# HueCodes/sudoku-vision

Measured on AMD Instinct MI355X. Metric: end-to-end frames/sec (1080p->81 digits), higher is better.
Workload: dtype f32

## Files before the change

sudoku-vision_amd/csrc/k3_cnn.hip:

```cpp
#include <cstring>

#include "sv_device.h"
#include "sv_internal.h"

typedef float f32x4 __attribute__((ext_vector_type(4)));
typedef float f32x2 __attribute__((ext_vector_type(2)));

namespace {

constexpr int PLANE = 257;
constexpr int C1_CELL = 32 * PLANE;
constexpr int IN_W = 30, IN_CELL = 900;
constexpr int FEAT = 3136;

__device__ __forceinline__ float glue_norm(u8 c) { return sv_glue_norm(c); }

struct N1Scratch {
    float cf[784];
    float rw[784];
    unsigned bits[16][8];
    unsigned pre[16][8];
    int residual[16], step[16];
};

// ... 794 lines not shown
    __shared__ N1Scratch sc[4];
    __shared__ float tile[4][IN_CELL];
    const int lane = threadIdx.x & 63, wave = threadIdx.x >> 6;
    const long c = (long)blockIdx.x * 4 + wave;
    if (c >= B) return;
    n1_preprocess_cell(cells + c * 784, tile[wave], sc[wave], lane, taps.k);
    wave_lds_fence();
    for (int i = lane; i < 784; i += 64) {
        const int y = i / 28, x = i - 28 * y;
        out[c * 784 + i] = tile[wave][(y + 1) * IN_W + x + 1] < 0.f ? 255 : 0;
    }
}

}

int svk_pack_weights_f32mfma(sv_weights &w, const float *c2w, const float *f1w)
{
    std::vector<float> w2(2 * 2 * 72 * 64);
    for (int np = 0; np < 2; np++)
        for (int t = 0; t < 2; t++)
            for (int ks = 0; ks < 72; ks++)
                for (int lane = 0; lane < 64; lane++) {
                    const int oc = 32 * np + 16 * t + (lane & 15), tap = ks >> 3, ic = (ks & 7) + 8 * (lane >> 4);
                    w2[((np * 2 + t) * 72 + ks) * 64 + lane] = c2w[(oc * 32 + ic) * 9 + tap];
                }
    std::vector<float> f1((size_t)196 * 8 * 64 * 4);
    for (int c = 0; c < 196; c++)
        for (int t = 0; t < 8; t++)
            for (int lane = 0; lane < 64; lane++)
                for (int e = 0; e < 4; e++) {
                    const int kp = 16 * c + 4 * (lane >> 4) + e, win = kp >> 6, oc = kp & 63, n = 16 * t + (lane & 15);
                    f1[(((size_t)c * 8 + t) * 64 + lane) * 4 + e] = f1w[(size_t)n * 3136 + oc * 49 + win];
                }
    int rc;
    if ((rc = sv_upload(w, &w.conv2_wreg, w2.data(), w2.size()))) return rc;
    if ((rc = sv_upload(w, &w.fc1_wreg, f1.data(), f1.size()))) return rc;
#ifdef SV_XCHECK
    std::vector<float> wino((size_t)4 * 16 * 8 * 64);
    std::vector<uint16_t> wsplit((size_t)4 * 16 * 3 * 64 * 8);
    const double G[4][3] = {{1, 0, 0}, {0.5, 0.5, 0.5}, {0.5, -0.5, 0.5}, {0, 0, 1}};
    for (int oc = 0; oc < 64; oc++)
        for (int ic = 0; ic < 32; ic++) {
            const float *g = c2w + (oc * 32 + ic) * 9;
            double Gg[4][3], U[4][4];
            for (int i = 0; i < 4; i++)
                for (int j = 0; j < 3; j++) Gg[i][j] = G[i][0] * g[j] + G[i][1] * g[3 + j] + G[i][2] * g[6 + j];
            for (int i = 0; i < 4; i++)
                for (int j = 0; j < 4; j++) U[i][j] = Gg[i][0] * G[j][0] + Gg[i][1] * G[j][1] + Gg[i][2] * G[j][2];
            const int nt = oc >> 4, lane = (oc & 15) + 16 * (ic & 3), ks = ic >> 2;
            for (int xi = 0; xi < 16; xi++) {
                const float u = (float)U[xi >> 2][xi & 3];
                wino[(((size_t)nt * 16 + xi) * 8 + ks) * 64 + lane] = u;
                float rest = u;
                for (int part = 0; part < 3; part++) {
                    uint32_t bits;
                    memcpy(&bits, &rest, 4);
                    bits &= 0xffff0000u;
                    float piece;
                    memcpy(&piece, &bits, 4);
                    rest -= piece;
                    wsplit[((((size_t)nt * 16 + xi) * 3 + part) * 64 + (oc & 15) + 16 * (ic >> 3)) * 8 + (ic & 7)] = (uint16_t)(bits >> 16);
                }
            }
        }
    if ((rc = sv_upload(w, &w.conv2_wino, wino.data(), wino.size()))) return rc;
    if ((rc = sv_upload(w, &w.conv2_wsplit, wsplit.data(), wsplit.size()))) return rc;
#endif
    return SV_OK;
}

int svk_preprocess_cells(const u8 *cells, long B, u8 *out, hipStream_t s)
{
    GaussTaps taps;
    sv_gaussian_taps_f32(11, taps.k);
    hipLaunchKernelGGL(k_preprocess_cells, dim3((unsigned)((B + 3) / 4)), dim3(256), 0, s, cells, B, taps, out);
    SV_LAUNCH_CHECK("k_preprocess_cells");
    return SV_OK;
}

__global__ __launch_bounds__(256) void k_softmax_topk(const float *__restrict__ logits, long B, int k, u8 *__restrict__ index, float *__restrict__ prob)
{
    const long cell = (long)blockIdx.x * 256 + threadIdx.x;
    if (cell >= B) return;
    float p[10];
    float best = -INFINITY;
#pragma unroll
    for (int j = 0; j < 10; j++) { p[j] = logits[cell * 10 + j]; best = fmaxf(best, p[j]); }
    float den = 0.f;
#pragma unroll
    for (int j = 0; j < 10; j++) { p[j] = expf(p[j] - best); den += p[j]; }
    unsigned taken = 0;
    for (int r = 0; r < k; r++) {
        float top = -1.f;
        int arg = 0;
#pragma unroll
        for (int j = 0; j < 10; j++)
            if (!(taken >> j & 1) && p[j] > top) { top = p[j]; arg = j; }
        taken |= 1u << arg;
        index[cell * k + r] = (u8)arg;
        prob[cell * k + r] = top / den;
    }
}

int svk_softmax_topk(const float *logits, long B, int k, u8 *index, float *prob, hipStream_t s)
{
    hipLaunchKernelGGL(k_softmax_topk, dim3((unsigned)((B + 255) / 256)), dim3(256), 0, s, logits, B, k, index, prob);
    SV_LAUNCH_CHECK("k_softmax_topk");
    return SV_OK;
}

static sv_cnn_algo effective_algo(const sv_ctx *ctx)
{
    switch (ctx->cnn_kernels) {
    case SV_CNN_F16PAIR: return SV_ALGO_F16PAIR;
    case SV_CNN_F32MFMA: return SV_ALGO_F32MFMA;
#ifdef SV_XCHECK
    case SV_CNN_X_WINOGRAD: return SV_ALGO_X_WINOGRAD;
    case SV_CNN_X_WSPLIT: return SV_ALGO_X_WSPLIT;
#endif
    default: return ctx->w.h2_in_range ? SV_ALGO_F16PAIR : SV_ALGO_F32MFMA;
    }
}

extern "C" int sv_ctx_set_cnn_kernels(sv_ctx *ctx, int which)
{
    if (!ctx) return sv_fail(SV_ERR_BAD_ARG, "sv_ctx_set_cnn_kernels: NULL context");
    bool ok = which == SV_CNN_AUTO || which == SV_CNN_F16PAIR || which == SV_CNN_F32MFMA;
#ifdef SV_XCHECK
    ok = ok || which == SV_CNN_X_WINOGRAD || which == SV_CNN_X_WSPLIT;
#endif
    if (!ok) return sv_fail(SV_ERR_BAD_ARG, "sv_ctx_set_cnn_kernels: unknown selection %d", which);
    ctx->cnn_kernels = which;
    return SV_OK;
}

#ifdef SV_XCHECK
extern "C" int svx_ctx_set_fc_frame_kernel(sv_ctx *ctx, int on)
{
    if (!ctx) return sv_fail(SV_ERR_BAD_ARG, "svx_ctx_set_fc_frame_kernel: NULL context");
    ctx->x_fc_frame = on != 0;
    return SV_OK;
}
#endif

extern "C" int sv_conv_kernel_info(sv_ctx *ctx, int *algo, int *mfma_f32_conv2_per_cell, int *mfma_f32_conv1_per_cell, int *mfma_f16_conv_per_cell,
                                   int *mfma_f16_fc_per_cell)
{
    if (!ctx || !algo || !mfma_f32_conv2_per_cell || !mfma_f32_conv1_per_cell || !mfma_f16_conv_per_cell || !mfma_f16_fc_per_cell)
        return sv_fail(SV_ERR_BAD_ARG, "sv_conv_kernel_info: NULL argument");
    const sv_cnn_algo a = effective_algo(ctx);
    *algo = a;
    *mfma_f32_conv2_per_cell = a == SV_ALGO_X_WINOGRAD ? 1568 : (a == SV_ALGO_F32MFMA ? 3600 : 0);
    *mfma_f32_conv1_per_cell = 0;
    *mfma_f16_conv_per_cell = a == SV_ALGO_F16PAIR ? 13 * 9 * 4 * 3 + 13 * 8 * 2 : 0;
    *mfma_f16_fc_per_cell = a == SV_ALGO_F16PAIR ? 98 * 8 * 3 / 16 : 0;
    return SV_OK;
}

__global__ __launch_bounds__(256) void k_input_range(const float *__restrict__ x, long n, float lo, float hi, int *__restrict__ flag)
{
    __shared__ float part[4];
    float m = 0.f;
    bool bad = false;
    for (long i = (long)blockIdx.x * 256 + threadIdx.x; i < n; i += (long)gridDim.x * 256) {
        const float v = fabsf(x[i]);
        bad |= !(v <= hi);
        m = fmaxf(m, v);
    }
    for (int d = 32; d > 0; d >>= 1) m = fmaxf(m, __shfl_xor(m, d));
    if ((threadIdx.x & 63) == 0) part[threadIdx.x >> 6] = m;
    if (__any(bad) && (threadIdx.x & 63) == 0) atomicOr(flag, 1);
    __syncthreads();
    if (threadIdx.x == 0) {
        m = fmaxf(fmaxf(part[0], part[1]), fmaxf(part[2], part[3]));
        if (m >= lo) atomicOr(flag + 1, 1);
    }
}
__global__ void k_input_range_finish(int *flag)
{
    if (flag[1] == 0) flag[0] = 1;
}

int svk_cnn_forward(sv_ctx *ctx, const void *x, bool x_is_u8, int glue, long B, float *logits, u8 *digits, float *conf, hipStream_t s)
{
    const sv_weights &w = ctx->w;
    const long npairs = (B + 1) / 2;
    if (ctx->precision == SV_PREC_BF16 && !x_is_u8)
        return sv_fail(SV_ERR_UNSUPPORTED, "sv_cnn_forward_f32: the bf16 configuration takes 8-bit cells (sv_cnn_forward_cells_u8 / sv_frames_to_digits)");
    if (x_is_u8 && glue == SV_GLUE_RUNPY) {
        int rc = svk_preprocess_cells((const u8 *)x, B, ctx->cells2, s);
        if (rc) return rc;
        x = ctx->cells2;
    }
    if (ctx->precision == SV_PREC_BF16) return svk_cnn_forward_bf16(ctx, (const u8 *)x, B, logits, digits, conf, s);
    sv_cnn_algo conv_algo = effective_algo(ctx);
    if (x_is_u8 && ((uintptr_t)x & 3)) conv_algo = SV_ALGO_F32MFMA;
    const int *flag = nullptr;
    if (conv_algo == SV_ALGO_F16PAIR && !x_is_u8 && ctx->cnn_kernels == SV_CNN_AUTO) {
        if (!ctx->range_flag) SV_HIP(hipMalloc((void **)&ctx->range_flag, 2 * sizeof(int)));
        SV_HIP(hipMemsetAsync(ctx->range_flag, 0, 2 * sizeof(int), s));
        const long n = B * 784;
        hipLaunchKernelGGL(k_input_range, dim3((unsigned)(n / 4096 + 1 < 1024 ? n / 4096 + 1 : 1024)), dim3(256), 0, s, (const float *)x, n, w.h2_x_lo, w.h2_x_hi, ctx->range_flag);
        hipLaunchKernelGGL(k_input_range_finish, dim3(1), dim3(1), 0, s, ctx->range_flag);
        SV_LAUNCH_CHECK("k_input_range");
        flag = ctx->range_flag;
    }
    if (conv_algo == SV_ALGO_F16PAIR) {
        const int rc = svk_cnn_forward_h2(ctx, x, x_is_u8, B, logits, digits, conf, flag, s);
        if (rc || !flag) return rc;
    }
#ifdef SV_XCHECK
    if (conv_algo == SV_ALGO_X_WSPLIT || conv_algo == SV_ALGO_X_WINOGRAD) {
        long cpw = (B + ctx->num_cus - 1) / ctx->num_cus;
        if (cpw < 1) cpw = 1;
        const int grid_s = (int)((B + cpw - 1) / cpw);
        sv_time_scope ts(ctx, SVK_CONV_FEATURES, s);
        if (conv_algo == SV_ALGO_X_WSPLIT) {
            if (x_is_u8)
                hipLaunchKernelGGL(k_conv_features_wsplit<true>, dim3(grid_s), dim3(512), 0, s, x, B, cpw, w.conv1_w, w.conv1_b, (const uint4 *)w.conv2_wsplit, w.conv2_b, ctx->features);
            else
                hipLaunchKernelGGL(k_conv_features_wsplit<false>, dim3(grid_s), dim3(512), 0, s, x, B, cpw, w.conv1_w, w.conv1_b, (const uint4 *)w.conv2_wsplit, w.conv2_b, ctx->features);
        } else {
            if (x_is_u8)
                hipLaunchKernelGGL(k_conv_features_wstream<true>, dim3(grid_s), dim3(512), 0, s, x, B, cpw, w.conv1_w, w.conv1_b, w.conv2_wino, w.conv2_b, ctx->features);
            else
                hipLaunchKernelGGL(k_conv_features_wstream<false>, dim3(grid_s), dim3(512), 0, s, x, B, cpw, w.conv1_w, w.conv1_b, w.conv2_wino, w.conv2_b, ctx->features);
        }
    } else
#endif
    {
        const int grid_pc = (int)(npairs < (long)ctx->num_cus ? npairs : (long)ctx->num_cus);
        sv_time_scope ts(ctx, SVK_CONV_FEATURES, s);
        if (x_is_u8)
            hipLaunchKernelGGL(k_conv_features_pc<true>, dim3(grid_pc), dim3(512), 0, s, x, B, w.conv1_w, w.conv1_b, w.conv2_wreg, w.conv2_b, ctx->features, flag);
        else
            hipLaunchKernelGGL(k_conv_features_pc<false>, dim3(grid_pc), dim3(512), 0, s, x, B, w.conv1_w, w.conv1_b, w.conv2_wreg, w.conv2_b, ctx->features, flag);
    }
    SV_LAUNCH_CHECK("k_conv_features");
    sv_time_scope ts(ctx, SVK_FC_HEAD, s);
#ifdef SV_XCHECK
    if (ctx->x_fc_frame && B >= 81 * 64)
        hipLaunchKernelGGL(k_fc_head_frame, dim3((unsigned)((B + 80) / 81)), dim3(512), 0, s, ctx->features, B, w.fc1_wreg, w.fc1_b, w.fc2_w, w.fc2_b, logits, digits, conf, flag);
    else
#endif
    hipLaunchKernelGGL(k_fc_head, dim3((unsigned)((B + 63) / 64)), dim3(256), 0, s, ctx->features, B, w.fc1_wreg, w.fc1_b, w.fc2_w, w.fc2_b, logits, digits, conf, flag);
    SV_LAUNCH_CHECK("k_fc_head");
    return SV_OK;
}
```

sudoku-vision_amd/csrc/k3_cnn_h2.hip:

```cpp
#include "sv_device.h"
#include "sv_internal.h"

typedef float f32x4 __attribute__((ext_vector_type(4)));
typedef float f32x2 __attribute__((ext_vector_type(2)));
typedef _Float16 h8 __attribute__((ext_vector_type(8)));

namespace {

constexpr int POS_STRIDE = 64, ROW_STRIDE = 16 * POS_STRIDE + 32;
constexpr int PLANE_B = 16 * ROW_STRIDE;
constexpr int IN_PLANE_B = 32 * 64;
constexpr int FEAT = 3136;

__device__ __forceinline__ float glue_norm(u8 c)
{
    const float t = __fdiv_rn((float)(255 - (int)c), 255.0f);
    return __fdiv_rn(__fsub_rn(t, 0.5f), 0.5f);
}

__device__ __forceinline__ void settle(uint4 &v) { asm volatile("" : "+v"(v.x), "+v"(v.y), "+v"(v.z), "+v"(v.w)); }
__device__ __forceinline__ void settle(float &v) { asm volatile("" : "+v"(v)); }

__device__ __forceinline__ unsigned pack2h(_Float16 a, _Float16 b)
{
    return (unsigned)__builtin_bit_cast(unsigned short, a) | ((unsigned)__builtin_bit_cast(unsigned short, b) << 16);
}

__host__ __device__ __forceinline__ void split_h2(float v, _Float16 &hi, _Float16 &lo)
{
    hi = (_Float16)v;
    lo = (_Float16)(v - (float)hi);
}

template <bool U8IN>
__global__ __launch_bounds__(512, 2) void k_conv_features_h2(const void *__restrict__ xin, long B, const uint4 *__restrict__ w1img,
                                                             const float *__restrict__ b1, float scale1_inv, const uint4 *__restrict__ w2img,
                                                             const float *__restrict__ b2, float scale_inv, float *__restrict__ feat, const int *__restrict__ run_if_clear
#ifdef SV_DEV
                                                             , int ablate
#endif
                                                             )
{
#ifndef SV_DEV
    constexpr int ablate = 0;
#endif
    if (run_if_clear && *run_if_clear != 0) return;
    __shared__ __attribute__((aligned(16))) unsigned char c1[2][2 * PLANE_B];
    __shared__ __attribute__((aligned(16))) unsigned char inh[2][2][IN_PLANE_B];
    __shared__ __attribute__((aligned(8))) unsigned short lut_in[208], lut_out[208];

    const int tid = threadIdx.x, lane = tid & 63;
    const int wave = __builtin_amdgcn_readfirstlane(tid >> 6);
    const bool consumer = wave < 4;
    const int c16 = lane & 15, q = lane >> 4;

    for (int i = tid; i < 4 * PLANE_B / 4; i += 512) ((unsigned *)c1)[i] = 0;
    for (int i = tid; i < 4 * IN_PLANE_B / 4; i += 512) ((unsigned *)inh)[i] = 0;
    for (int g = tid; g < 208; g += 512) {
        const int gc = g < 196 ? g : 195, wy = gc / 14, wx = gc - 14 * wy;
        lut_in[g] = (unsigned short)((2 * wy) * 64 + 4 * wx);
        lut_out[g] = (unsigned short)((wy + 1) * ROW_STRIDE + (wx + 1) * POS_STRIDE);
    }
    __syncthreads();

    const long first = blockIdx.x, stride = gridDim.x;
    const long ncell = first < B ? (B - first + stride - 1) / stride : 0;
    if (ncell == 0) return;

    if (!consumer) {
        __builtin_amdgcn_s_setprio(1);
        const int ptid = tid & 255;
        unsigned sraw[4] = {0, 0, 0, 0};
        auto stage_load = [&](long c) {
            if (U8IN) {
                if (ptid < 196) sraw[0] = ((const unsigned *)((const u8 *)xin + c * 784))[ptid];
            } else {
#pragma unroll
                for (int j = 0; j < 4; j++)
                    if (ptid + 256 * j < 784) sraw[j] = __float_as_uint(((const float *)xin)[c * 784 + ptid + 256 * j]);
            }
        };
        auto put = [&](int slot, int y, int x, float v) {
            _Float16 h, l;
            split_h2(v, h, l);
            unsigned char *d = inh[slot][0] + (y + 1) * 64 + (x + 1) * 2;
            *(_Float16 *)d = h;
            *(_Float16 *)(d + IN_PLANE_B) = l;
        };
        auto stage_store = [&](int slot) {
            if (U8IN) {
                if (ptid < 196) {
                    const int y = ptid / 7, x = 4 * (ptid - 7 * y);
#pragma unroll
                    for (int j = 0; j < 4; j++) put(slot, y, x + j, glue_norm((u8)(sraw[0] >> (8 * j))));
                }
            } else {
#pragma unroll
                for (int j = 0; j < 4; j++) {
                    const int i = ptid + 256 * j;
                    if (i < 784) { const int y = i / 28; put(slot, y, i - y * 28, __uint_as_float(sraw[j])); }
                }
            }
        };
        const int chalf = (wave >> 1) & 1, ppar = (wave & 1) ^ 1;
        uint4 b1reg[4][2];
#pragma unroll
        for (int pos = 0; pos < 4; pos++)
#pragma unroll
            for (int m = 0; m < 2; m++) b1reg[pos][m] = w1img[((chalf * 4 + pos) * 2 + m) * 64 + lane];
        float bias1 = b1[16 * chalf + c16];
#pragma unroll
        for (int pos = 0; pos < 4; pos++) { settle(b1reg[pos][0]); settle(b1reg[pos][1]); }
        settle(bias1);
        stage_load(first);
        stage_store(0);
        __syncthreads();
        const int ntile1 = (ablate & 1) ? 0 : (ppar ? 6 : 7);
        for (long k = 0; k < ncell; k++) {
            if (k + 1 < ncell) stage_load(first + (k + 1) * stride);
            const unsigned char *src_part = inh[k & 1][q >> 1] + 2 * (q & 1) * 64;
            unsigned char *dst_cell = c1[k & 1] + (16 * chalf + c16) * 2;
            f32x4 acc[2][4];
            auto fetch_mfma = [&](int j, int set) {
                const unsigned *src = (const unsigned *)(src_part + lut_in[16 * j + c16]);
                const uint4 araw = {src[0], src[1], src[16], src[17]};
                const h8 a = __builtin_bit_cast(h8, araw);
#pragma unroll
                for (int pos = 0; pos < 4; pos++) {
                    acc[set][pos] = __builtin_amdgcn_mfma_f32_16x16x32_f16(a, __builtin_bit_cast(h8, b1reg[pos][0]), (f32x4){0.f, 0.f, 0.f, 0.f}, 0, 0, 0);
                    acc[set][pos] = __builtin_amdgcn_mfma_f32_16x16x32_f16(a, __builtin_bit_cast(h8, b1reg[pos][1]), acc[set][pos], 0, 0, 0);
                }
            };
            auto finish = [&](int j, int set) {
                const uint2 oo = *(const uint2 *)&lut_out[16 * j + 4 * q];
#pragma unroll
                for (int reg = 0; reg < 4; reg++) {
                    const float m = fmaxf(fmaxf(acc[set][0][reg], acc[set][1][reg]), fmaxf(acc[set][2][reg], acc[set][3][reg]));
                    const float v = fmaxf(__builtin_fmaf(m, scale1_inv, bias1), 0.f);
                    _Float16 h, l;
                    split_h2(v, h, l);
                    const unsigned off = ((reg & 2) ? oo.y : oo.x) >> (16 * (reg & 1)) & 0xFFFFu;
                    *(_Float16 *)(dst_cell + off) = h;
                    *(_Float16 *)(dst_cell + off + PLANE_B) = l;
                }
            };
            if (ntile1 > 0) fetch_mfma(ppar, 0);
#pragma unroll
            for (int jj = 1; jj < 7; jj++) {
                if (jj >= ntile1) break;
                fetch_mfma(ppar + 2 * jj, jj & 1);
                finish(ppar + 2 * (jj - 1), (jj - 1) & 1);
            }
            if (ntile1 > 0) finish(ppar + 2 * (ntile1 - 1), (ntile1 - 1) & 1);
            if (k + 1 < ncell) stage_store((k + 1) & 1);
            __syncthreads();
        }
        __syncthreads();
        return;
    }

    const int np = wave >> 1, par = wave & 1;
    uint4 breg[9][2][2];
#pragma unroll
    for (int tap = 0; tap < 9; tap++)
#pragma unroll
        for (int t = 0; t < 2; t++)
#pragma unroll
            for (int p = 0; p < 2; p++) breg[tap][t][p] = w2img[(((tap * 2 + np) * 2 + t) * 2 + p) * 64 + lane];
    float bias2_0 = b2[32 * np + 2 * c16], bias2_1 = b2[32 * np + 2 * c16 + 1];
#pragma unroll
    for (int tap = 0; tap < 9; tap++)
#pragma unroll
        for (int t = 0; t < 2; t++) { settle(breg[tap][t][0]); settle(breg[tap][t][1]); }
    settle(bias2_0);
    settle(bias2_1);
    __syncthreads();
    __syncthreads();
    constexpr int PF = 5, RING = 6;
    uint4 ring_h[RING], ring_l[RING];
    unsigned tile_off[7];
#pragma unroll
    for (int jj = 0; jj < 7; jj++) {
        int g = 4 * (par + 2 * jj) + (c16 >> 2);
        if (g > 48) g = 48;
        const int wy = g / 7, wx = g - 7 * wy, sp = c16 & 3;
        tile_off[jj] = (unsigned)((2 * wy + (sp >> 1)) * ROW_STRIDE + (2 * wx + (sp & 1)) * POS_STRIDE + q * 16);
    }
#define SV_TAP_OFF(tap) (((tap) / 3) * ROW_STRIDE + ((tap) % 3) * POS_STRIDE)
#define SV_SLOT() __builtin_amdgcn_sched_barrier(0)
    const int ntile = (ablate & 2) ? 0 : (par ? 6 : 7);
    const unsigned out_off = (32 * par + 8 * q + 4 * np + (c16 >> 2)) * 32 + (c16 & 3) * 4;
    unsigned long long dbg_t[4] = {0, 0, 0, 0}, dbg_s = 0;
#define SV_STAMP(i) do { if (ablate & 16) { unsigned long long t_ = __builtin_amdgcn_s_memtime(); __builtin_amdgcn_s_waitcnt(0xC07F); dbg_t[i] += t_ - dbg_s; dbg_s = t_; } } while (0)
    if (ablate & 16) dbg_s = __builtin_amdgcn_s_memtime();
    for (long k = 0; k < ncell; k++) {
        SV_STAMP(0);
        const char *fcell = (const char *)(feat + (first + k * stride) * FEAT);
        const unsigned char *cbase = c1[k & 1];
        const unsigned char *ap = cbase + tile_off[0], *ap_next = ap;
#pragma unroll
        for (int st = 0; st < PF; st++) {
            ring_h[st % RING] = *(const uint4 *)(ap + SV_TAP_OFF(st));
            ring_l[st % RING] = *(const uint4 *)(ap + SV_TAP_OFF(st) + PLANE_B);
        }
        f32x4 acc[2][2];
        float m0 = 0.f, m1 = 0.f, t0 = 0.f, t1 = 0.f;
        unsigned hp = 0, lp = 0;
        auto epilogue = [&](int piece, int jp, int set) {
            const f32x4 &v0 = acc[set][0], &v1 = acc[set][1];
            switch (piece) {
            case 0: asm volatile("v_max3_f32 %0, %1, %2, %3" : "=v"(m0) : "v"(v0[0]), "v"(v0[1]), "v"(v0[2])); break;
            case 1: asm volatile("v_max3_f32 %0, %1, %2, %3" : "=v"(m1) : "v"(v1[0]), "v"(v1[1]), "v"(v1[2])); break;
            case 2: asm volatile("v_max_f32 %0, %0, %1" : "+v"(m0) : "v"(v0[3])); break;
            case 3: asm volatile("v_max_f32 %0, %0, %1" : "+v"(m1) : "v"(v1[3])); break;
            case 4: asm volatile("v_fma_f32 %0, %0, %1, %2" : "+v"(m0) : "s"(scale_inv), "v"(bias2_0)); break;
            case 5: asm volatile("v_fma_f32 %0, %0, %1, %2" : "+v"(m1) : "s"(scale_inv), "v"(bias2_1)); break;
            case 6: asm volatile("v_max_f32 %0, 0, %0" : "+v"(m0)); break;
            case 7: asm volatile("v_max_f32 %0, 0, %0" : "+v"(m1)); break;
            case 8: asm volatile("v_cvt_pk_f16_f32 %0, %1, %2" : "=v"(hp) : "v"(m0), "v"(m1)); break;
            case 9: asm volatile("v_fma_mix_f32 %0, %1, -1.0, %2 op_sel:[0,0,0] op_sel_hi:[1,0,0]" : "=v"(t0) : "v"(hp), "v"(m0)); break;
            case 10: asm volatile("v_fma_mix_f32 %0, %1, -1.0, %2 op_sel:[1,0,0] op_sel_hi:[1,0,0]" : "=v"(t1) : "v"(hp), "v"(m1)); break;
            case 11: asm volatile("v_cvt_pk_f16_f32 %0, %1, %2" : "=v"(lp) : "v"(t0), "v"(t1)); break;
            case 12:
                if (jp < 6 || q == 0) *(unsigned *)(fcell + jp * 2048 + out_off) = hp;
                break;
            case 13:
                if (jp < 6 || q == 0) *(unsigned *)(fcell + jp * 2048 + out_off + 16) = lp;
                break;
            default: break;
            }
        };
#pragma unroll
        for (int jj = 0; jj < 7; jj++) {
            if (jj >= ntile) break;
            const int set = jj & 1;
#pragma unroll
            for (int tap = 0; tap < 9; tap++) {
                const int st = jj * 9 + tap;
                const bool pf_here = tap + PF < 9, pf_next = !pf_here && jj + 1 < ntile;
                const unsigned char *pa = pf_here ? ap + SV_TAP_OFF((tap + PF) % 9) : ap_next + SV_TAP_OFF((tap + PF) % 9);
                const h8 ah = __builtin_bit_cast(h8, ring_h[st % RING]), al = __builtin_bit_cast(h8, ring_l[st % RING]);
                const h8 bh0 = __builtin_bit_cast(h8, breg[tap][0][0]), bl0 = __builtin_bit_cast(h8, breg[tap][0][1]);
                const h8 bh1 = __builtin_bit_cast(h8, breg[tap][1][0]), bl1 = __builtin_bit_cast(h8, breg[tap][1][1]);
                const int e0 = (jj > 0 && tap >= 2 && tap <= 6 && 3 * (tap - 2) < 14) ? 3 * (tap - 2) : -1;
                SV_SLOT();
                if (tap == 0) asm volatile("v_mfma_f32_16x16x32_f16 %0, %1, %2, 0" : "=&v"(acc[set][0]) : "v"(ah), "v"(bh0));
                else asm volatile("v_mfma_f32_16x16x32_f16 %0, %1, %2, %0" : "+v"(acc[set][0]) : "v"(ah), "v"(bh0));
                if (pf_here || pf_next) ring_h[(st + PF) % RING] = *(const uint4 *)pa;
                SV_SLOT();
                if (tap == 0) asm volatile("v_mfma_f32_16x16x32_f16 %0, %1, %2, 0" : "=&v"(acc[set][1]) : "v"(ah), "v"(bh1));
                else asm volatile("v_mfma_f32_16x16x32_f16 %0, %1, %2, %0" : "+v"(acc[set][1]) : "v"(ah), "v"(bh1));
                if (tap == 1 && jj + 1 < ntile) ap_next = cbase + tile_off[jj + 1 < 7 ? jj + 1 : 6];
                SV_SLOT();
                asm volatile("v_mfma_f32_16x16x32_f16 %0, %1, %2, %0" : "+v"(acc[set][0]) : "v"(ah), "v"(bl0));
                if (pf_here || pf_next) ring_l[(st + PF) % RING] = *(const uint4 *)(pa + PLANE_B);
                SV_SLOT();
                asm volatile("v_mfma_f32_16x16x32_f16 %0, %1, %2, %0" : "+v"(acc[set][1]) : "v"(ah), "v"(bl1));
                if (e0 >= 0) epilogue(e0, jj - 1, set ^ 1);
                SV_SLOT();
                asm volatile("v_mfma_f32_16x16x32_f16 %0, %1, %2, %0" : "+v"(acc[set][0]) : "v"(al), "v"(bh0));
                if (e0 >= 0) epilogue(e0 + 1, jj - 1, set ^ 1);
                SV_SLOT();
                asm volatile("v_mfma_f32_16x16x32_f16 %0, %1, %2, %0" : "+v"(acc[set][1]) : "v"(al), "v"(bh1));
                if (e0 >= 0) epilogue(e0 + 2, jj - 1, set ^ 1);
                SV_SLOT();
            }
            ap = ap_next;
        }
        SV_STAMP(1);
        if (ntile > 0) {
            asm volatile("s_nop 15\n\ts_nop 15");
#pragma unroll
            for (int piece = 0; piece < 14; piece++) epilogue(piece, ntile - 1, (ntile - 1) & 1);
        }
        SV_STAMP(2);
        __syncthreads();
        SV_STAMP(3);
    }
    if ((ablate & 16) && blockIdx.x < 2 && lane == 0)
        printf("blk %d wave %d ncell %ld: loop-top %llu tiles %llu epilogue %llu barrier %llu cycles/cell\n", (int)blockIdx.x, wave, ncell, dbg_t[0] / ncell, dbg_t[1] / ncell,
               dbg_t[2] / ncell, dbg_t[3] / ncell);
#undef SV_SLOT
#undef SV_TAP_OFF
}

__global__ __launch_bounds__(256, 2) void k_fc_head_h2(const float *__restrict__ feat, long B, const uint4 *__restrict__ w1img,
                                                       const float *__restrict__ b1, float scale_inv, const float *__restrict__ w2,
                                                       const float *__restrict__ b2, float *__restrict__ logits,
                                                       u8 *__restrict__ digits, float *__restrict__ conf, const int *__restrict__ run_if_clear)
{
    if (run_if_clear && *run_if_clear != 0) return;
// ... 123 lines not shown
#pragma unroll
        for (int i = 0; i < 2; i++) {
            const int rl = prow + 4 * i;
            long row = base + rl;
            if (row >= c_end) row = c_end - 1;
            const unsigned gr = ((unsigned)(rl & 3) << 2) | ((unsigned)(rl >> 2) & 3u);
            asrc[i] = (const unsigned char *)feat + row * (FEAT * 4) + (((unsigned)pslot) ^ gr) * 16;
        }
        const uint4 *wp = w1img + (wave & 7) * 4 * 64 + lane;
        auto issue_w = [&](int st) {
            if (loader) {
                const unsigned dst = lds_base + (st & 1) * FCP_W_STAGE + (wave & 7) * 4096;
#pragma unroll
                for (int j = 0; j < 4; j++) fcp_glds(wp + (long)st * 2048 + 64 * j, dst + 1024 * j);
            }
        };
        auto issue_a = [&](int st) {
            const unsigned dst = lds_base + FCP_OFF_A + (st % 3) * FCP_A_STAGE + 2 * wave * 1024;
#pragma unroll
            for (int i = 0; i < 2; i++) fcp_glds(asrc[i] + 256 * st, dst + 1024 * i);
        };
        f32x4 acc_h[4], acc_l[4];
#pragma unroll
        for (int t = 0; t < 4; t++) { acc_h[t] = (f32x4){0.f, 0.f, 0.f, 0.f}; acc_l[t] = (f32x4){0.f, 0.f, 0.f, 0.f}; }
        issue_w(0);
        issue_a(0);
        issue_a(1);

        auto compute = [&](int st) {
            constexpr int BD = 4;
            const unsigned char *wt = lds + (st & 1) * FCP_W_STAGE + lane * 16, *at = lds + (st % 3) * FCP_A_STAGE;
            uint4 fa[4], fb[8][2];
#pragma unroll
            for (int c = 0; c < 4; c++) fa[c] = *(const uint4 *)(at + a_off[c]);
            auto rd = [&](int i) {
                const int sstep = i >> 2, t = i & 3;
                fb[i][0] = *(const uint4 *)(wt + ((sstep * 8 + 4 * nh + t) * 2 + 0) * 1024);
                fb[i][1] = *(const uint4 *)(wt + ((sstep * 8 + 4 * nh + t) * 2 + 1) * 1024);
            };
#pragma unroll
            for (int i = 0; i < BD; i++) rd(i);
            __builtin_amdgcn_sched_barrier(0);
            const h8 ah[2] = {__builtin_bit_cast(h8, fa[0]), __builtin_bit_cast(h8, fa[2])}, al[2] = {__builtin_bit_cast(h8, fa[1]), __builtin_bit_cast(h8, fa[3])};
#pragma unroll
            for (int i = 0; i < 8; i += 2) {
                if (i + BD < 8) { rd(i + BD); rd(i + BD + 1); }
                __builtin_amdgcn_sched_barrier(0);
                const int sstep = i >> 2, t = i & 3;
                const h8 bh0 = __builtin_bit_cast(h8, fb[i][0]), bl0 = __builtin_bit_cast(h8, fb[i][1]);
                const h8 bh1 = __builtin_bit_cast(h8, fb[i + 1][0]), bl1 = __builtin_bit_cast(h8, fb[i + 1][1]);
                acc_h[t] = __builtin_amdgcn_mfma_f32_16x16x32_f16(ah[sstep], bh0, acc_h[t], 0, 0, 0);
                acc_h[t + 1] = __builtin_amdgcn_mfma_f32_16x16x32_f16(ah[sstep], bh1, acc_h[t + 1], 0, 0, 0);
                acc_l[t] = __builtin_amdgcn_mfma_f32_16x16x32_f16(ah[sstep], bl0, acc_l[t], 0, 0, 0);
                acc_l[t + 1] = __builtin_amdgcn_mfma_f32_16x16x32_f16(ah[sstep], bl1, acc_l[t + 1], 0, 0, 0);
                acc_l[t] = __builtin_amdgcn_mfma_f32_16x16x32_f16(al[sstep], bh0, acc_l[t], 0, 0, 0);
                acc_l[t + 1] = __builtin_amdgcn_mfma_f32_16x16x32_f16(al[sstep], bh1, acc_l[t + 1], 0, 0, 0);
                __builtin_amdgcn_sched_barrier(0);
            }
        };
        for (int st = 0; st < FCP_NSTAGE; st++) {
            if (st + 1 < FCP_NSTAGE) asm volatile("s_waitcnt vmcnt(2)" ::: "memory"); else asm volatile("s_waitcnt vmcnt(0)" ::: "memory");
            __builtin_amdgcn_s_barrier();
            asm volatile("" ::: "memory");
            if (st + 1 < FCP_NSTAGE) issue_w(st + 1);
            if (st + 2 < FCP_NSTAGE) issue_a(st + 2);
            if (tile_live) compute(st);
        }
        __syncthreads();

#pragma unroll
        for (int t = 0; t < 4; t++) {
            const float bias = b1[64 * nh + 16 * t + r];
#pragma unroll
            for (int reg = 0; reg < 4; reg++)
                hs[16 * mt + 4 * q + reg][64 * nh + 16 * t + r] = fmaxf((acc_h[t][reg] + acc_l[t][reg]) * scale_inv + bias, 0.f);
        }
        __syncthreads();
        if (nh == 0) {
            for (int jj = 0; jj < 3; jj++) {
                const int j = q + 4 * jj;
                if (j < 10) {
                    const float s = sv_fc2_logit(hs[16 * mt + r], w2s, b2, j);
                    lg[mt][r][j] = s;
                    if (cell0 + r < c_end) logits[(cell0 + r) * 10 + j] = s;
                }
            }
        }
        __syncthreads();
        if (nh == 0 && q == 0 && cell0 + r < c_end) sv_digit_conf(lg[mt][r], cell0 + r, digits, conf);
    }
}

}

int svk_pack_weights_h2(sv_weights &w, const float *c1w, const float *c1b, const float *c2w, const float *c2b, const float *f1w)
{
    int eA = 0, eF = 0;
    {
        auto row_sum_max = [](const float *wt, int rows, int cols) { double m = 0; for (int r = 0; r < rows; r++) { double a = 0; for (int c = 0; c < cols; c++) a += std::fabs((double)wt[(size_t)r * cols + c]); m = std::fmax(m, a); } return m; };
        auto abs_max = [](const float *v, int n) { double m = 0; for (int i = 0; i < n; i++) m = std::fmax(m, std::fabs((double)v[i])); return m; };
        const double LIM = 6.0e4, A1 = row_sum_max(c1w, 32, 9), B1 = abs_max(c1b, 32), A2 = row_sum_max(c2w, 64, 288), B2 = abs_max(c2b, 64);
        const double U1 = A1 + B1, U2 = A2 * U1 + B2;
        if (U1 > 0 && U1 < 1) eA = std::min(-std::ilogb(U1), 120);
        if (U2 > 0 && U2 < 1) eF = std::min(-std::ilogb(U2), 120);
        const double sA = std::ldexp(1.0, eA), sF = std::ldexp(1.0, eF);
        double hi = LIM;
        if (A1 > 0) hi = std::fmin(hi, (LIM / sA - B1) / A1);
        else if (B1 * sA > LIM) hi = -1;
        if (A2 > 0 && A1 > 0) hi = std::fmin(hi, ((LIM / sF - B2) / A2 - B1) / A1);
        else if ((A2 * B1 + B2) * sF > LIM) hi = -1;
        if (!std::isfinite(A1) || !std::isfinite(A2) || !std::isfinite(B1) || !std::isfinite(B2) || !(hi == hi)) hi = -1;
        w.h2_x_hi = (float)hi;
        w.h2_x_lo = 0x1p-3f;
        w.h2_in_range = hi >= 1.0;
    }
    auto pow2_scale = [](const float *v, size_t n) -> int {
        float m = 0.f;
        for (size_t i = 0; i < n; i++) m = std::fmax(m, std::fabs(v[i]));
        if (!(m > 0.f) || !std::isfinite(m)) return 0;
        const int e = 13 - std::ilogb(m);
        return e > 120 ? 120 : e;
    };
    auto split_bits = [](float ws, uint16_t &hi, uint16_t &lo) {
        _Float16 h, l;
        split_h2(ws, h, l);
        hi = __builtin_bit_cast(uint16_t, h);
        lo = __builtin_bit_cast(uint16_t, l);
    };
    const int e2 = pow2_scale(c2w, 18432), e1 = pow2_scale(f1w, 401408);
    const float s2 = std::ldexp(1.f, e2), s1 = std::ldexp(1.f, e1);
    w.conv2_h2_scale_inv = std::ldexp(1.f, eF - eA - e2);
    w.fc1_h2_scale_inv = std::ldexp(1.f, -eF - e1);
    std::vector<uint16_t> c2h((size_t)9 * 2 * 2 * 2 * 64 * 8), f1h((size_t)98 * 8 * 2 * 64 * 8);
    for (int tap = 0; tap < 9; tap++)
        for (int np = 0; np < 2; np++)
            for (int t = 0; t < 2; t++)
                for (int lane = 0; lane < 64; lane++)
                    for (int j = 0; j < 8; j++) {
                        const int oc = 32 * np + 2 * (lane & 15) + t, ic = 8 * (lane >> 4) + j;
                        const size_t base = ((((size_t)tap * 2 + np) * 2 + t) * 2) * 64 * 8;
                        split_bits(c2w[(oc * 32 + ic) * 9 + tap] * s2, c2h[base + (size_t)lane * 8 + j], c2h[base + 512 + (size_t)lane * 8 + j]);
                    }
    for (int st = 0; st < 98; st++)
        for (int t = 0; t < 8; t++)
            for (int lane = 0; lane < 64; lane++)
                for (int j = 0; j < 8; j++) {
                    const int kp = 64 * (st >> 1) + 16 * (lane >> 4) + 8 * (st & 1) + j, win = kp >> 6, oc = kp & 63, n = 16 * t + (lane & 15);
                    const size_t base = (((size_t)st * 8 + t) * 2) * 64 * 8;
                    split_bits(f1w[(size_t)n * 3136 + oc * 49 + win] * s1, f1h[base + (size_t)lane * 8 + j], f1h[base + 512 + (size_t)lane * 8 + j]);
                }
    const int e0 = pow2_scale(c1w, 288);
    const float s0 = std::ldexp(1.f, e0);
    w.conv1_h2_scale_inv = std::ldexp(1.f, eA - e0);
    for (int e : {eA - e0, eF - eA - e2, -eF - e1})
        if (e < -126 || e > 127) w.h2_in_range = false;
    std::vector<float> c1bs(c1b, c1b + 32), c2bs(c2b, c2b + 64);
    for (float &b : c1bs) b = std::ldexp(b, eA);
    for (float &b : c2bs) b = std::ldexp(b, eF);
    std::vector<uint16_t> c1h((size_t)2 * 4 * 2 * 64 * 8);
    for (int chalf = 0; chalf < 2; chalf++)
        for (int pos = 0; pos < 4; pos++)
            for (int lane = 0; lane < 64; lane++)
                for (int j = 0; j < 8; j++) {
                    const int kk = 8 * (lane >> 4) + j, part = kk >> 4, pp = kk & 15, r = pp >> 2, c = pp & 3;
                    const int ky = r - (pos >> 1), kx = c - (pos & 1), ch = 16 * chalf + (lane & 15);
                    uint16_t hi = 0, lo = 0;
                    if (ky >= 0 && ky < 3 && kx >= 0 && kx < 3) split_bits(c1w[ch * 9 + ky * 3 + kx] * s0, hi, lo);
                    const size_t base = (((size_t)chalf * 4 + pos) * 2) * 64 * 8 + (size_t)lane * 8 + j;
                    c1h[base] = hi;
                    c1h[base + 512] = part == 0 ? lo : 0;
                }
    int rc;
    if ((rc = sv_upload(w, &w.conv1_h2, c1h.data(), c1h.size()))) return rc;
    if ((rc = sv_upload(w, &w.conv2_h2, c2h.data(), c2h.size()))) return rc;
    if ((rc = sv_upload(w, &w.fc1_h2, f1h.data(), f1h.size()))) return rc;
    if ((rc = sv_upload(w, &w.conv1_b_h2, c1bs.data(), c1bs.size()))) return rc;
    return sv_upload(w, &w.conv2_b_h2, c2bs.data(), c2bs.size());
}

#ifdef SV_DEV
extern "C" int sv_dev_set_h2_ablate(sv_ctx *ctx, int bits) { if (!ctx) return SV_ERR_BAD_ARG; ctx->dev_ablate = bits; return SV_OK; }
#endif

int svk_cnn_forward_h2(sv_ctx *ctx, const void *x, bool x_is_u8, long B, float *logits, u8 *digits, float *conf, const int *run_if_clear, hipStream_t s)
{
    const sv_weights &w = ctx->w;
    const int grid = (int)(B < (long)ctx->num_cus ? B : (long)ctx->num_cus);
#ifdef SV_DEV
#define SV_ABLATE_ARG , ctx->dev_ablate
#else
#define SV_ABLATE_ARG
#endif
    {
        sv_time_scope ts(ctx, SVK_CONV_FEATURES, s);
        if (x_is_u8)
            hipLaunchKernelGGL(k_conv_features_h2<true>, dim3(grid), dim3(512), 0, s, x, B, (const uint4 *)w.conv1_h2, w.conv1_b_h2, w.conv1_h2_scale_inv, (const uint4 *)w.conv2_h2, w.conv2_b_h2,
                               w.conv2_h2_scale_inv, ctx->features, run_if_clear SV_ABLATE_ARG);
        else
            hipLaunchKernelGGL(k_conv_features_h2<false>, dim3(grid), dim3(512), 0, s, x, B, (const uint4 *)w.conv1_h2, w.conv1_b_h2, w.conv1_h2_scale_inv, (const uint4 *)w.conv2_h2, w.conv2_b_h2,
                               w.conv2_h2_scale_inv, ctx->features, run_if_clear SV_ABLATE_ARG);
    }
#undef SV_ABLATE_ARG
    SV_LAUNCH_CHECK("k_conv_features_h2");
    sv_time_scope ts(ctx, SVK_FC_HEAD, s);
    const long per = std::max<long>(16, (B + ctx->num_cus - 1) / ctx->num_cus);
    if (per <= FCP_CELLS) {
        hipLaunchKernelGGL(k_fc_head_h2p, dim3((unsigned)((B + per - 1) / per)), dim3(64 * FCP_WAVES), 0, s, ctx->features, B, per, (const uint4 *)w.fc1_h2, w.fc1_b,
                           w.fc1_h2_scale_inv, w.fc2_w, w.fc2_b, logits, digits, conf, run_if_clear);
        SV_LAUNCH_CHECK("k_fc_head_h2p");
        return SV_OK;
    }
    hipLaunchKernelGGL(k_fc_head_h2, dim3((unsigned)((B + 63) / 64)), dim3(256), 0, s, ctx->features, B, (const uint4 *)w.fc1_h2, w.fc1_b, w.fc1_h2_scale_inv,
                       w.fc2_w, w.fc2_b, logits, digits, conf, run_if_clear);
    SV_LAUNCH_CHECK("k_fc_head_h2");
    return SV_OK;
}
```

sudoku-vision_amd/csrc/sv_internal.h:

```cpp
#pragma once
#include <hip/hip_runtime.h>
#include <cstdarg>
#include <cstdint>
#include <cstdio>
#include <vector>

#include "../../include/sudoku_vision_hip.h"
#ifdef SV_XCHECK
#include "../../include/sudoku_vision_xcheck.h"
#endif

typedef uint8_t u8;

struct sv_weights {
    float *conv1_w = nullptr;
    float *conv1_b = nullptr;
    float *conv2_wreg = nullptr;
    float *conv2_wino = nullptr;
    float *conv2_b = nullptr;
    float *fc1_wreg = nullptr;
    float *fc1_b = nullptr;
    unsigned short *conv2_wsplit = nullptr;
    unsigned short *conv2_bf16 = nullptr;
    unsigned short *fc1_bf16 = nullptr;
    unsigned short *conv2_h2 = nullptr;
    unsigned short *fc1_h2 = nullptr;
    unsigned short *conv1_h2 = nullptr;
    float conv1_h2_scale_inv = 1.f, conv2_h2_scale_inv = 1.f, fc1_h2_scale_inv = 1.f;
    float *conv1_b_h2 = nullptr;
    float *conv2_b_h2 = nullptr;
    bool h2_in_range = true;
    float h2_x_lo = 0.f, h2_x_hi = 0.f;
    float *fc2_w = nullptr;
    float *fc2_b = nullptr;
    bool loaded = false;
    std::vector<void *> allocs;
};

struct sv_conv3 { float *w = nullptr, *b = nullptr; };
struct sv_weights3 {
    sv_conv3 stem, conv1[5], conv2[5], shortcut[5];
    float *se1[5] = {}, *se2[5] = {};
    float *fc_w = nullptr, *fc_b = nullptr;
    float temperature = 1.f;
    bool use_se = true, loaded = false;
    std::vector<void *> allocs;
};

struct sv_ctx {
    int device = 0;
    int num_cus = 256;
    sv_weights w;
    sv_weights3 w3;
    float *v3_act = nullptr;
    long cap_v3 = 0;
    float *features = nullptr;
    u8 *cells = nullptr;
    u8 *cells2 = nullptr;
    long cap_cells = 0;
    u8 *jpeg_planes = nullptr;
    size_t cap_jpeg = 0;
    u8 *pp2 = nullptr;
    size_t cap_pp2 = 0;
    void *k1_list = nullptr;
    int precision = 0;
    int cnn_kernels = 0;
    int *range_flag = nullptr;
    bool x_fc_frame = false;
    int dev_ablate = 0;
    bool timing = false;
    struct timed { int kernel; hipEvent_t t0, t1; };
    std::vector<timed> timeline;
    std::vector<hipEvent_t> event_pool;
};

enum sv_kernel_id { SVK_PREPROCESS = 0, SVK_WARP_CELLS = 1, SVK_CONV_FEATURES = 2, SVK_FC_HEAD = 3, SVK_FUSED12 = 4, SVK_COUNT = 5 };

struct sv_time_scope {
    sv_ctx *ctx; hipStream_t s; int idx = -1;
    sv_time_scope(sv_ctx *c, int kernel, hipStream_t st);
    ~sv_time_scope();
};

int sv_fail(int code, const char *fmt, ...);

#define SV_HIP(expr)                                                                         \
    do {                                                                                     \
        hipError_t e_ = (expr);                                                              \
        if (e_ != hipSuccess) return sv_fail(SV_ERR_HIP, "%s: %s", #expr, hipGetErrorString(e_)); \
    } while (0)

#define SV_LAUNCH_CHECK(name)                                                                \
    do {                                                                                     \
        hipError_t e_ = hipGetLastError();                                                   \
        if (e_ != hipSuccess) return sv_fail(SV_ERR_HIP, "launch %s: %s", name, hipGetErrorString(e_)); \
    } while (0)

int sv_ensure_scratch(sv_ctx *ctx, long cells);

template <class T>
int sv_upload(sv_weights &w, T **dst, const T *src, size_t n)
{
    SV_HIP(hipMalloc((void **)dst, n * sizeof(T)));
    w.allocs.push_back(*dst);
    SV_HIP(hipMemcpy(*dst, src, n * sizeof(T), hipMemcpyHostToDevice));
    return SV_OK;
}

enum sv_cnn_algo { SV_ALGO_F32MFMA = 0, SV_ALGO_X_WINOGRAD = 2, SV_ALGO_X_WSPLIT = 3, SV_ALGO_F16PAIR = 4 };

int svk_gray(const u8 *bgr, int n, int H, int W, ptrdiff_t pitch, ptrdiff_t img_stride, u8 *gray, hipStream_t s);
int svk_blur(const u8 *src, int n, int H, int W, int ksize, u8 *dst, hipStream_t s);
int svk_adaptive_threshold(const u8 *src, int n, int H, int W, int block, const float *taps, int idelta, int type_inv,
                           u8 *dst, hipStream_t s);
int svk_preprocess(sv_ctx *ctx, const u8 *bgr, int n, int H, int W, ptrdiff_t pitch, ptrdiff_t img_stride, u8 *binary, hipStream_t s);
int svk_preprocess_bits(sv_ctx *ctx, const u8 *bgr, int n, int H, int W, ptrdiff_t pitch, ptrdiff_t img_stride, uint32_t *bits, hipStream_t s);
int svk_despeckle_bits(uint32_t *bits, int n, int H, int W, hipStream_t s);
int svk_preprocess_mm_stats(sv_ctx *ctx, unsigned *ambiguous, unsigned long *capacity);
int svk_preprocess_mm_enable_stats(sv_ctx *ctx);
bool svk_preprocess_mm_supported(const u8 *bgr, int H, int W, ptrdiff_t pitch, ptrdiff_t img_stride, const void *out, bool bits);
int svk_preprocess_mm(sv_ctx *ctx, const u8 *bgr, int n, int H, int W, ptrdiff_t pitch, ptrdiff_t img_stride, u8 *out, bool bits, float *mean_dbg, hipStream_t s);
int svk_preprocess_warp_fused(sv_ctx *ctx, const u8 *bgr, int n, int H, int W, ptrdiff_t pitch, ptrdiff_t img_stride, u8 *binary, const double *minv, u8 *cells,
                              hipStream_t s);
int svk_warp_perspective(const u8 *img, int H, int W, ptrdiff_t pitch, int channels, const double *minv, int out_size,
                         u8 *dst, hipStream_t s);
int svk_extract_cells(const u8 *grid, int h, int w, ptrdiff_t pitch, int channels, int cell_size, int margin_h,
                      int margin_w, u8 *cells, hipStream_t s);
int svk_warp_cells(sv_ctx *ctx, const u8 *frames, int n, int H, int W, ptrdiff_t pitch, ptrdiff_t frame_stride, const double *minv,
                   u8 *cells, hipStream_t s);
int svk_cnn_forward(sv_ctx *ctx, const void *x, bool x_is_u8, int glue, long B, float *logits, u8 *digits, float *conf,
                    hipStream_t s);
int svk_pack_weights_f32mfma(sv_weights &w, const float *c2w, const float *f1w);
int svk_pack_weights_bf16(sv_weights &w, const float *c2w, const float *f1w);
int svk_pack_weights_h2(sv_weights &w, const float *c1w, const float *c1b, const float *c2w, const float *c2b, const float *f1w);

int svk_despeckle(const u8 *src, int n, int H, int W, u8 *dst, unsigned *packed, hipStream_t s);
int svk_pack_sparse_bits(const uint32_t *bits, int n, int H, int W, u8 *records, long stride, hipStream_t s);
int svk_copy_to_host(const void *src, void *dst_host, size_t bytes, hipStream_t s);
int svk_resize_linear(const u8 *src, int sh, int sw, ptrdiff_t pitch, u8 *dst, int dh, int dw, hipStream_t s);
int svk_cnn_forward_bf16(sv_ctx *ctx, const u8 *cells, long B, float *logits, u8 *digits, float *conf, hipStream_t s);
int svk_cnn_forward_h2(sv_ctx *ctx, const void *x, bool x_is_u8, long B, float *logits, u8 *digits, float *conf, const int *run_if_clear, hipStream_t s);
int svk_cell_ink_ratio(const u8 *cells, long B, int npx, float *ratio, int *otsu, hipStream_t s);
int svk_preprocess_cells(const u8 *cells, long B, u8 *out, hipStream_t s);
int svk_jpeg_reconstruct(sv_ctx *ctx, const sv_jpeg_info *info, const int16_t *coef, const uint64_t *masks, const uint32_t *offsets, const int16_t *values,
                         const uint16_t *quant, u8 *bgr, ptrdiff_t pitch, hipStream_t s);
int svk_softmax_topk(const float *logits, long B, int k, u8 *index, float *prob, hipStream_t s);
int svk_frame_quality_stats(const u8 *img, int n, int H, int W, ptrdiff_t pitch, ptrdiff_t img_stride, int C, long long *lap_sum, long long *lap_sqsum,
                            uint32_t *hist, hipStream_t s);
int svk_grid_line_coverage(const void *src, bool bits, int n, int H, int W, ptrdiff_t pitch, ptrdiff_t img_stride, const double *minv, uint32_t *counts,
                           hipStream_t s);
int svk_morphology(sv_ctx *ctx, const u8 *src, int n, int H, int W, ptrdiff_t pitch, ptrdiff_t img_stride, int op, int shape, int k, u8 *dst, hipStream_t s);
int svk_box_mean(const u8 *src, int n, int H, int W, ptrdiff_t pitch, ptrdiff_t img_stride, int k, u8 *dst, hipStream_t s);
int svk_threshold_sauvola(const u8 *src, int n, int H, int W, ptrdiff_t pitch, ptrdiff_t img_stride, int window, double k, u8 *dst, hipStream_t s);
int svk_gaussian_blur21(const u8 *src, int n, int H, int W, ptrdiff_t pitch, ptrdiff_t img_stride, u8 *dst, hipStream_t s);
int svk_clahe(sv_ctx *ctx, const u8 *src, int n, int H, int W, ptrdiff_t pitch, ptrdiff_t img_stride, double clip, int tiles_x, int tiles_y, u8 *dst, hipStream_t s);
int svk_divide_normalize(const u8 *gray, int n, int H, int W, ptrdiff_t pitch, ptrdiff_t img_stride, const u8 *background, u8 *dst, hipStream_t s);
int svk_threshold_count(const u8 *src, int n, int H, int W, ptrdiff_t pitch, ptrdiff_t img_stride, int thresh, int type_inv, u8 *dst, uint32_t *counts, hipStream_t s);
int svk_shadow_mask(const u8 *gray, int n, int H, int W, ptrdiff_t pitch, ptrdiff_t img_stride, const u8 *local_mean, int delta, u8 *mask, uint32_t *counts, hipStream_t s);
int svk_count_nonzero(const u8 *src, int n, int H, int W, ptrdiff_t pitch, ptrdiff_t img_stride, uint32_t *counts, hipStream_t s);

int svk_pack_weights_v3(sv_weights3 &w, const float *blob, bool use_se);
long svk_v3_blob_floats(bool use_se);
size_t svk_v3_scratch_bytes(long cells);
int svk_cnn3_forward(sv_ctx *ctx, const void *x, bool x_is_u8, long B, float *logits, float *features, u8 *digits, float *conf, hipStream_t s);

void sv_gaussian_taps_f32(int n, float *out);
```

Measured before the change: 206,500.

## Feed conv1 exact integer u8 inputs as single fp16 plane, halving conv1 MFMAs

For u8 inputs, conv1 now stores each pixel as the exact integer 255-2c in one fp16 plane instead of a hi/lo split of the normalized float. The 1/255 normalization is folded into a two-part scale (scale_inv plus scale_lo) applied after accumulation. This halves the conv1 MFMAs per position and the input shared-memory traffic. To support it, a separate conv1 weight image is built whose hi/lo parts sit in the K dimension. The change relies on the integer inputs being exact in fp16 and on the folded scale staying within range.

```diff
diff --git a/sudoku-vision_amd/csrc/k3_cnn.hip b/sudoku-vision_amd/csrc/k3_cnn.hip
--- a/sudoku-vision_amd/csrc/k3_cnn.hip
+++ b/sudoku-vision_amd/csrc/k3_cnn.hip
@@ -970,7 +970,7 @@
     *algo = a;
     *mfma_f32_conv2_per_cell = a == SV_ALGO_X_WINOGRAD ? 1568 : (a == SV_ALGO_F32MFMA ? 3600 : 0);
     *mfma_f32_conv1_per_cell = 0;
-    *mfma_f16_conv_per_cell = a == SV_ALGO_F16PAIR ? 13 * 9 * 4 * 3 + 13 * 8 * 2 : 0;
+    *mfma_f16_conv_per_cell = a == SV_ALGO_F16PAIR ? 13 * 9 * 4 * 3 + 13 * 8 * 1 : 0;
     *mfma_f16_fc_per_cell = a == SV_ALGO_F16PAIR ? 98 * 8 * 3 / 16 : 0;
     return SV_OK;
 }
diff --git a/sudoku-vision_amd/csrc/k3_cnn_h2.hip b/sudoku-vision_amd/csrc/k3_cnn_h2.hip
--- a/sudoku-vision_amd/csrc/k3_cnn_h2.hip
+++ b/sudoku-vision_amd/csrc/k3_cnn_h2.hip
@@ -12,12 +12,6 @@
 constexpr int IN_PLANE_B = 32 * 64;
 constexpr int FEAT = 3136;
 
-__device__ __forceinline__ float glue_norm(u8 c)
-{
-    const float t = __fdiv_rn((float)(255 - (int)c), 255.0f);
-    return __fdiv_rn(__fsub_rn(t, 0.5f), 0.5f);
-}
-
 __device__ __forceinline__ void settle(uint4 &v) { asm volatile("" : "+v"(v.x), "+v"(v.y), "+v"(v.z), "+v"(v.w)); }
 __device__ __forceinline__ void settle(float &v) { asm volatile("" : "+v"(v)); }
 
@@ -34,7 +28,7 @@
 
 template <bool U8IN>
 __global__ __launch_bounds__(512, 2) void k_conv_features_h2(const void *__restrict__ xin, long B, const uint4 *__restrict__ w1img,
-                                                             const float *__restrict__ b1, float scale1_inv, const uint4 *__restrict__ w2img,
+                                                             const float *__restrict__ b1, float scale1_inv, float scale1_lo, const uint4 *__restrict__ w2img,
                                                              const float *__restrict__ b2, float scale_inv, float *__restrict__ feat, const int *__restrict__ run_if_clear
 #ifdef SV_DEV
                                                              , int ablate
@@ -46,7 +40,8 @@
 #endif
     if (run_if_clear && *run_if_clear != 0) return;
     __shared__ __attribute__((aligned(16))) unsigned char c1[2][2 * PLANE_B];
-    __shared__ __attribute__((aligned(16))) unsigned char inh[2][2][IN_PLANE_B];
+    constexpr int NPL = U8IN ? 1 : 2;
+    __shared__ __attribute__((aligned(16))) unsigned char inh[2][NPL][IN_PLANE_B];
     __shared__ __attribute__((aligned(8))) unsigned short lut_in[208], lut_out[208];
 
     const int tid = threadIdx.x, lane = tid & 63;
@@ -55,7 +50,7 @@
     const int c16 = lane & 15, q = lane >> 4;
 
     for (int i = tid; i < 4 * PLANE_B / 4; i += 512) ((unsigned *)c1)[i] = 0;
-    for (int i = tid; i < 4 * IN_PLANE_B / 4; i += 512) ((unsigned *)inh)[i] = 0;
+    for (int i = tid; i < 2 * NPL * IN_PLANE_B / 4; i += 512) ((unsigned *)inh)[i] = 0;
     for (int g = tid; g < 208; g += 512) {
         const int gc = g < 196 ? g : 195, wy = gc / 14, wx = gc - 14 * wy;
         lut_in[g] = (unsigned short)((2 * wy) * 64 + 4 * wx);
@@ -85,14 +80,19 @@
             split_h2(v, h, l);
             unsigned char *d = inh[slot][0] + (y + 1) * 64 + (x + 1) * 2;
             *(_Float16 *)d = h;
-            *(_Float16 *)(d + IN_PLANE_B) = l;
+            *(_Float16 *)(d + (NPL - 1) * IN_PLANE_B) = l;
         };
         auto stage_store = [&](int slot) {
             if (U8IN) {
                 if (ptid < 196) {
                     const int y = ptid / 7, x = 4 * (ptid - 7 * y);
-#pragma unroll
-                    for (int j = 0; j < 4; j++) put(slot, y, x + j, glue_norm((u8)(sraw[0] >> (8 * j))));
+                    _Float16 qh[4];
+#pragma unroll
+                    for (int j = 0; j < 4; j++) qh[j] = (_Float16)(255 - 2 * (int)((sraw[0] >> (8 * j)) & 255u));
+                    unsigned char *d = inh[slot][0] + (y + 1) * 64 + (x + 1) * 2;
+                    *(_Float16 *)d = qh[0];
+                    *(unsigned *)(d + 2) = pack2h(qh[1], qh[2]);
+                    *(_Float16 *)(d + 6) = qh[3];
                 }
             } else {
 #pragma unroll
@@ -103,14 +103,14 @@
             }
         };
         const int chalf = (wave >> 1) & 1, ppar = (wave & 1) ^ 1;
-        uint4 b1reg[4][2];
+        uint4 b1reg[4][NPL];
 #pragma unroll
         for (int pos = 0; pos < 4; pos++)
 #pragma unroll
-            for (int m = 0; m < 2; m++) b1reg[pos][m] = w1img[((chalf * 4 + pos) * 2 + m) * 64 + lane];
+            for (int m = 0; m < NPL; m++) b1reg[pos][m] = w1img[((chalf * 4 + pos) * NPL + m) * 64 + lane];
         float bias1 = b1[16 * chalf + c16];
 #pragma unroll
-        for (int pos = 0; pos < 4; pos++) { settle(b1reg[pos][0]); settle(b1reg[pos][1]); }
+        for (int pos = 0; pos < 4; pos++) { settle(b1reg[pos][0]); settle(b1reg[pos][NPL - 1]); }
         settle(bias1);
         stage_load(first);
         stage_store(0);
@@ -118,7 +118,7 @@
         const int ntile1 = (ablate & 1) ? 0 : (ppar ? 6 : 7);
         for (long k = 0; k < ncell; k++) {
             if (k + 1 < ncell) stage_load(first + (k + 1) * stride);
-            const unsigned char *src_part = inh[k & 1][q >> 1] + 2 * (q & 1) * 64;
+            const unsigned char *src_part = inh[k & 1][U8IN ? 0 : q >> 1] + 2 * (q & 1) * 64;
             unsigned char *dst_cell = c1[k & 1] + (16 * chalf + c16) * 2;
             f32x4 acc[2][4];
             auto fetch_mfma = [&](int j, int set) {
@@ -128,7 +128,7 @@
 #pragma unroll
                 for (int pos = 0; pos < 4; pos++) {
                     acc[set][pos] = __builtin_amdgcn_mfma_f32_16x16x32_f16(a, __builtin_bit_cast(h8, b1reg[pos][0]), (f32x4){0.f, 0.f, 0.f, 0.f}, 0, 0, 0);
-                    acc[set][pos] = __builtin_amdgcn_mfma_f32_16x16x32_f16(a, __builtin_bit_cast(h8, b1reg[pos][1]), acc[set][pos], 0, 0, 0);
+                    if (!U8IN) acc[set][pos] = __builtin_amdgcn_mfma_f32_16x16x32_f16(a, __builtin_bit_cast(h8, b1reg[pos][NPL - 1]), acc[set][pos], 0, 0, 0);
                 }
             };
             auto finish = [&](int j, int set) {
@@ -136,7 +136,7 @@
 #pragma unroll
                 for (int reg = 0; reg < 4; reg++) {
                     const float m = fmaxf(fmaxf(acc[set][0][reg], acc[set][1][reg]), fmaxf(acc[set][2][reg], acc[set][3][reg]));
-                    const float v = fmaxf(__builtin_fmaf(m, scale1_inv, bias1), 0.f);
+                    const float v = fmaxf(__builtin_fmaf(m, scale1_inv, U8IN ? __builtin_fmaf(m, scale1_lo, bias1) : bias1), 0.f);
                     _Float16 h, l;
                     split_h2(v, h, l);
                     const unsigned off = ((reg & 2) ? oo.y : oo.x) >> (16 * (reg & 1)) & 0xFFFFu;
@@ -566,12 +566,19 @@
     const int e0 = pow2_scale(c1w, 288);
     const float s0 = std::ldexp(1.f, e0);
     w.conv1_h2_scale_inv = std::ldexp(1.f, eA - e0);
+    const int e0q = std::min(e0, eA + 118);
+    const float s0q = std::ldexp(1.f, e0q);
+    {
+        const double f = std::ldexp(1.0, eA - e0q) / 255.0;
+        w.conv1_h2q_scale_inv = (float)f;
+        w.conv1_h2q_scale_lo = (float)(f - (double)w.conv1_h2q_scale_inv);
+    }
     for (int e : {eA - e0, eF - eA - e2, -eF - e1})
         if (e < -126 || e > 127) w.h2_in_range = false;
     std::vector<float> c1bs(c1b, c1b + 32), c2bs(c2b, c2b + 64);
     for (float &b : c1bs) b = std::ldexp(b, eA);
     for (float &b : c2bs) b = std::ldexp(b, eF);
-    std::vector<uint16_t> c1h((size_t)2 * 4 * 2 * 64 * 8);
+    std::vector<uint16_t> c1h((size_t)2 * 4 * 2 * 64 * 8), c1q((size_t)2 * 4 * 64 * 8);
     for (int chalf = 0; chalf < 2; chalf++)
         for (int pos = 0; pos < 4; pos++)
             for (int lane = 0; lane < 64; lane++)
@@ -583,9 +590,13 @@
                     const size_t base = (((size_t)chalf * 4 + pos) * 2) * 64 * 8 + (size_t)lane * 8 + j;
                     c1h[base] = hi;
                     c1h[base + 512] = part == 0 ? lo : 0;
+                    hi = lo = 0;
+                    if (ky >= 0 && ky < 3 && kx >= 0 && kx < 3) split_bits(c1w[ch * 9 + ky * 3 + kx] * s0q, hi, lo);
+                    c1q[(((size_t)chalf * 4 + pos) * 64 + lane) * 8 + j] = part == 0 ? hi : lo;
                 }
     int rc;
     if ((rc = sv_upload(w, &w.conv1_h2, c1h.data(), c1h.size()))) return rc;
+    if ((rc = sv_upload(w, &w.conv1_h2q, c1q.data(), c1q.size()))) return rc;
     if ((rc = sv_upload(w, &w.conv2_h2, c2h.data(), c2h.size()))) return rc;
     if ((rc = sv_upload(w, &w.fc1_h2, f1h.data(), f1h.size()))) return rc;
     if ((rc = sv_upload(w, &w.conv1_b_h2, c1bs.data(), c1bs.size()))) return rc;
@@ -608,11 +619,11 @@
     {
         sv_time_scope ts(ctx, SVK_CONV_FEATURES, s);
         if (x_is_u8)
-            hipLaunchKernelGGL(k_conv_features_h2<true>, dim3(grid), dim3(512), 0, s, x, B, (const uint4 *)w.conv1_h2, w.conv1_b_h2, w.conv1_h2_scale_inv, (const uint4 *)w.conv2_h2, w.conv2_b_h2,
-                               w.conv2_h2_scale_inv, ctx->features, run_if_clear SV_ABLATE_ARG);
+            hipLaunchKernelGGL(k_conv_features_h2<true>, dim3(grid), dim3(512), 0, s, x, B, (const uint4 *)w.conv1_h2q, w.conv1_b_h2, w.conv1_h2q_scale_inv, w.conv1_h2q_scale_lo,
+                               (const uint4 *)w.conv2_h2, w.conv2_b_h2, w.conv2_h2_scale_inv, ctx->features, run_if_clear SV_ABLATE_ARG);
         else
-            hipLaunchKernelGGL(k_conv_features_h2<false>, dim3(grid), dim3(512), 0, s, x, B, (const uint4 *)w.conv1_h2, w.conv1_b_h2, w.conv1_h2_scale_inv, (const uint4 *)w.conv2_h2, w.conv2_b_h2,
-                               w.conv2_h2_scale_inv, ctx->features, run_if_clear SV_ABLATE_ARG);
+            hipLaunchKernelGGL(k_conv_features_h2<false>, dim3(grid), dim3(512), 0, s, x, B, (const uint4 *)w.conv1_h2, w.conv1_b_h2, w.conv1_h2_scale_inv, 0.f,
+                               (const uint4 *)w.conv2_h2, w.conv2_b_h2, w.conv2_h2_scale_inv, ctx->features, run_if_clear SV_ABLATE_ARG);
     }
 #undef SV_ABLATE_ARG
     SV_LAUNCH_CHECK("k_conv_features_h2");
diff --git a/sudoku-vision_amd/csrc/sv_internal.h b/sudoku-vision_amd/csrc/sv_internal.h
--- a/sudoku-vision_amd/csrc/sv_internal.h
+++ b/sudoku-vision_amd/csrc/sv_internal.h
@@ -26,7 +26,9 @@
     unsigned short *conv2_h2 = nullptr;
     unsigned short *fc1_h2 = nullptr;
     unsigned short *conv1_h2 = nullptr;
+    unsigned short *conv1_h2q = nullptr;
     float conv1_h2_scale_inv = 1.f, conv2_h2_scale_inv = 1.f, fc1_h2_scale_inv = 1.f;
+    float conv1_h2q_scale_inv = 1.f, conv1_h2q_scale_lo = 0.f;
     float *conv1_b_h2 = nullptr;
     float *conv2_b_h2 = nullptr;
     bool h2_in_range = true;
```

Result: no change. 209,200 (median of 3 runs) (+1.3%).
